# pawanjay176/kzg_rust

Measured on AMD Instinct MI355X. Metric: blobs/sec on verify_blob_kzg_proof_batch (mainnet 4096, batch=64), higher is better.
Workload: dtype u32 limbs (29-bit) / 64-bit accumulate, u8 bytes

## Files before the change

__graft_entry__.py:

```python
import os
import subprocess
import sys

ROOT = os.path.dirname(os.path.abspath(__file__))
if ROOT not in sys.path:
    sys.path.insert(0, ROOT)


def build() -> None:
    env = dict(os.environ)
    subprocess.run(["make", "-C", os.path.join(ROOT, "kzg_rust_amd", "csrc"), "-j5"], check=True, env=env)
    subprocess.run(["make", "-C", os.path.join(ROOT, "oracle")], check=True, env=env)
    native = os.path.join(ROOT, "tests", "native")
    subprocess.run(["g++", "-O2", "-shared", "-fPIC", "-o", os.path.join(native, "libhd_probe.so"), os.path.join(native, "hd_probe.cpp")],
                   check=True, env=env)
    subprocess.run(["g++", "-O2", "-shared", "-fPIC", "-o", os.path.join(native, "liblazy_chain_probe.so"), os.path.join(native, "lazy_chain_probe.cpp")],
                   check=True, env=env)
    subprocess.run(["g++", "-O2", "-shared", "-fPIC", "-o", os.path.join(native, "libmont_columns_probe.so"), os.path.join(native, "mont_columns_probe.cpp")],
                   check=True, env=env)
    subprocess.run(["g++", "-O2", "-std=c++17", "-shared", "-fPIC", "-o", os.path.join(native, "liblc_forms_probe.so"), os.path.join(native, "lc_forms_probe.cpp")],
                   check=True, env=env)
    subprocess.run(["g++", "-std=c++17", "-O2", "-o", os.path.join(native, "cpp_vector_runner"), os.path.join(native, "cpp_vector_runner.cpp"),
                    "-L" + os.path.join(ROOT, "kzg_rust_amd"), "-lkzg355", "-Wl,-rpath," + os.path.join(ROOT, "kzg_rust_amd")], check=True, env=env)
    subprocess.run(["g++", "-std=c++17", "-O2", "-o", os.path.join(native, "cpp_cell_runner"), os.path.join(native, "cpp_cell_runner.cpp"),
                    "-L" + os.path.join(ROOT, "kzg_rust_amd"), "-lkzg355", "-Wl,-rpath," + os.path.join(ROOT, "kzg_rust_amd")], check=True, env=env)
    subprocess.run(["g++", "-std=c++17", "-O2", "-o", os.path.join(native, "cpp_cell_compute_runner"), os.path.join(native, "cpp_cell_compute_runner.cpp"),
                    "-L" + os.path.join(ROOT, "kzg_rust_amd"), "-lkzg355", "-Wl,-rpath," + os.path.join(ROOT, "kzg_rust_amd")], check=True, env=env)
    subprocess.run(["g++", "-std=c++17", "-O2", "-o", os.path.join(native, "cpp_cell_recover_runner"), os.path.join(native, "cpp_cell_recover_runner.cpp"),
                    "-L" + os.path.join(ROOT, "kzg_rust_amd"), "-lkzg355", "-Wl,-rpath," + os.path.join(ROOT, "kzg_rust_amd")], check=True, env=env)
    subprocess.run(["g++", "-std=c++17", "-O2", "-o", os.path.join(native, "cpp_cell_recover_sets_runner"), os.path.join(native, "cpp_cell_recover_sets_runner.cpp"),
                    "-L" + os.path.join(ROOT, "kzg_rust_amd"), "-lkzg355", "-Wl,-rpath," + os.path.join(ROOT, "kzg_rust_amd")], check=True, env=env)
    subprocess.run(["g++", "-std=c++17", "-O2", "-o", os.path.join(native, "cpp_blob_cell_runner"), os.path.join(native, "cpp_blob_cell_runner.cpp"),
                    "-L" + os.path.join(ROOT, "kzg_rust_amd"), "-lkzg355", "-Wl,-rpath," + os.path.join(ROOT, "kzg_rust_amd")], check=True, env=env)
    quad_src, quad_bin = os.path.join(native, "quad_ops_test.hip"), os.path.join(native, "quad_ops_test")
    quad_deps = [quad_src] + [os.path.join(ROOT, "kzg_rust_amd", "csrc", f) for f in ("g1_quad.h", "g1.h", "field.h", "modinv.h", "consts_gen.h")]
    if not os.path.exists(quad_bin) or any(os.path.getmtime(d) > os.path.getmtime(quad_bin) for d in quad_deps):
        subprocess.run(["/opt/rocm/bin/hipcc", "-O3", "-std=c++17", "--offload-arch=gfx950", "-Wno-unused-result", "-o", quad_bin, quad_src], check=True, env=env)
    probe_src, probe_so = os.path.join(native, "gpu_probe.hip"), os.path.join(native, "libgpu_probe.so")
    probe_deps = [probe_src] + [os.path.join(ROOT, "kzg_rust_amd", "csrc", f) for f in ("field.h", "modinv.h", "eval_core.h", "consts_gen.h")]
    if not os.path.exists(probe_so) or any(os.path.getmtime(d) > os.path.getmtime(probe_so) for d in probe_deps):
        subprocess.run(["/opt/rocm/bin/hipcc", "-O3", "-std=c++17", "--offload-arch=gfx950", "-Wno-unused-result", "-shared", "-fPIC", "-o", probe_so, probe_src],
                       check=True, env=env)
    group_src, group_so = os.path.join(native, "gpu_group_probe.hip"), os.path.join(native, "libgpu_group_probe.so")
    group_deps = [group_src] + [os.path.join(ROOT, "kzg_rust_amd", "csrc", f) for f in
                                ("field.h", "modinv.h", "tower.h", "g1.h", "pairing.h", "pairing_coop.h", "pairing_lanes.h", "consts_gen.h")]
    if not os.path.exists(group_so) or any(os.path.getmtime(d) > os.path.getmtime(group_so) for d in group_deps):
        subprocess.run(["/opt/rocm/bin/hipcc", "-O3", "-std=c++17", "--offload-arch=gfx950", "-Wno-unused-result", "-shared", "-fPIC", "-o", group_so, group_src],
                       check=True, env=env)
    import kzg_rust_amd
    from kzg_rust_amd import _lib
    lib = _lib.load()
    for name in _lib.EXPORTED_SYMBOLS:
        getattr(lib, name)
    print("build ok:", lib.kzg355_version().decode())


def smoke() -> None:
    import torch
    assert torch.cuda.is_available(), "smoke() needs a GPU"
    import kzg_rust_amd as kz
    from oracle.oracle import Oracle
    sys.path.insert(0, os.path.join(ROOT, "tests"))
    from synth import random_blob
    golden = os.path.join(ROOT, "tests", "golden")
    g1 = open(os.path.join(golden, "trusted_setup_g1.bin"), "rb").read()
    g2 = open(os.path.join(golden, "trusted_setup_g2.bin"), "rb").read()
    s = kz.Kzg.load_trusted_setup([g1[48 * i:48 * i + 48] for i in range(4096)], [g2[96 * i:96 * i + 96] for i in range(65)])
    o = Oracle()
    os_ = o.load_trusted_setup(g1, g2)
    blobs = [random_blob(1000 + i) for i in range(3)]
    cs = [kz.Kzg.blob_to_kzg_commitment(kz.Blob(b), s) for b in blobs]
    assert [c.to_bytes() for c in cs] == [o.blob_to_kzg_commitment(b, os_) for b in blobs], "commitment mismatch vs oracle"
    ps = [kz.Kzg.compute_blob_kzg_proof(kz.Blob(b), c, s) for b, c in zip(blobs, cs)]
    assert [p.to_bytes() for p in ps] == [o.compute_blob_kzg_proof(b, c.to_bytes(), os_) for b, c in zip(blobs, cs)], "proof mismatch vs oracle"
    ok = kz.Kzg.verify_blob_kzg_proof_batch([kz.Blob(b) for b in blobs], cs, ps, s)
    assert ok is True and o.verify_blob_kzg_proof_batch(blobs, [c.to_bytes() for c in cs], [p.to_bytes() for p in ps], os_) is True
    bad = [ps[1], ps[0], ps[2]]
    assert kz.Kzg.verify_blob_kzg_proof_batch([kz.Blob(b) for b in blobs], cs, bad, s) is False
    s.free()
    o.free_trusted_setup(os_)
    print("smoke ok: commit/prove bit-exact vs oracle, verify batch true/false as expected")


if __name__ == "__main__":
    build()
    if len(sys.argv) > 1 and sys.argv[1] == "smoke":
        smoke()
```

kzg_rust_amd/csrc/eval_core.h:

```cpp
#pragma once
#include "field.h"

namespace kzg {

struct EvalGroup { Fr sa, sb, st; };
constexpr int EVAL_ZPOWERS = 12;
constexpr int EVAL_WAVES = 4;
constexpr int EVAL_TAB_L1 = 0, EVAL_TAB_L2 = 1024, EVAL_TAB_L3 = 1280, EVAL_TAB_L4 = 1344, EVAL_TAB_L5 = 1360, EVAL_TAB_L6 = 1364, EVAL_TAB_GROUPS = 1365;
struct EvalPiece { uint32_t w[4]; };
constexpr int EVAL_TAB_PIECES = ((EVAL_TAB_GROUPS + 63) / 64) * 7 * 64;
KZG_HD constexpr int eval_tab_piece(int e, int q) { return (e / 64) * 7 * 64 + q * 64 + (e % 64); }
KZG_HD void eval_group_pack(EvalPiece p[7], const EvalGroup &g) {
    for (int k = 0; k < 28; k++) p[k / 4].w[k % 4] = k < NFR ? g.sa.l[k] : k < 2 * NFR ? g.sb.l[k - NFR] : k < 3 * NFR ? g.st.l[k - 2 * NFR] : 0u;
}
KZG_HD void eval_group_unpack(EvalGroup &g, const EvalPiece p[7]) {
#pragma unroll
    for (int k = 0; k < 27; k++) (k < NFR ? g.sa.l[k] : k < 2 * NFR ? g.sb.l[k - NFR] : g.st.l[k - 2 * NFR]) = p[k / 4].w[k % 4];
}
KZG_HD constexpr int eval_tab_first(int level) {
    return level == 1 ? EVAL_TAB_L1 : level == 2 ? EVAL_TAB_L2 : level == 3 ? EVAL_TAB_L3 : level == 4 ? EVAL_TAB_L4 : level == 5 ? EVAL_TAB_L5 : EVAL_TAB_L6;
}

template <int K> struct FrMultiple {
    uint32_t l[NFR];
    constexpr FrMultiple() : l{} {
        const uint32_t m[NFR] = FR_MOD_INIT;
        uint64_t c = 0;
        for (int i = 0; i < NFR; i++) { c += (uint64_t)m[i] * (uint32_t)K; l[i] = i < NFR - 1 ? (uint32_t)(c & LMASK) : (uint32_t)c; c >>= LB; }
    }
};
template <int K> KZG_HD void fr_sub_bias(Fr &r, const Fr &a, const Fr &b) {
    constexpr FrMultiple<K> kr;
    int32_t c = 0;
#pragma unroll
    for (int i = 0; i < NFR; i++) {
        const int32_t t = (int32_t)a.l[i] - (int32_t)b.l[i] + (int32_t)kr.l[i] + c;
        if (i < NFR - 1) { c = t >> LB; r.l[i] = (uint32_t)t & LMASK; }
        else r.l[i] = (uint32_t)t;
    }
}

KZG_HD void fr_add_raw(Fr &r, const Fr &a, const Fr &b) {
#pragma unroll
    for (int i = 0; i < NFR; i++) r.l[i] = a.l[i] + b.l[i];
}
template <int K> struct FrMultipleRaw {
    uint32_t l[NFR];
    constexpr FrMultipleRaw() : l{} {
        const FrMultiple<K> n;
        for (int i = 0; i < NFR; i++) l[i] = n.l[i] + (i < NFR - 1 ? (1u << LB) : 0u) - (i > 0 ? 1u : 0u);
    }
};
template <int K> KZG_HD void fr_sub_bias_raw(Fr &r, const Fr &a, const Fr &b) {
    constexpr FrMultipleRaw<K> kr;
#pragma unroll
    for (int i = 0; i < NFR; i++) r.l[i] = a.l[i] - b.l[i] + kr.l[i];
}
KZG_HD void fr_add_sweep(Fr &r, const Fr &a, const Fr &b) {
    uint32_t c = 0;
#pragma unroll
    for (int i = 0; i < NFR; i++) {
        const uint32_t t = a.l[i] + b.l[i] + c;
        if (i < NFR - 1) { c = t >> LB; r.l[i] = t & LMASK; } else r.l[i] = t;
    }
}

template <int K> KZG_HD void eval_node2(Fr &n, const Fr &n0, const Fr &n1, const Fr &zk, const Fr &s) {
    Fr A, B;
    fr_add_raw(A, n0, n1);
    fr_sub_bias_raw<K>(B, n0, n1);
    fr_mul2_lazy(n, A, zk, B, s);
}
KZG_HD void eval_group(Fr &n, const Fr c[4], const Fr &zk, const Fr &zk2, const EvalGroup &g) {
    Fr na, nb;
    eval_node2<2>(na, c[0], c[1], zk, g.sa);
    eval_node2<2>(nb, c[2], c[3], zk, g.sb);
    eval_node2<2>(n, na, nb, zk2, g.st);
}
KZG_HD void eval_group_leaves(Fr &n, Fr &Sp, const uint32_t pw[4][8], const Fr &z, const Fr &z2, const EvalGroup &g) {
    Fr p0, p1, p2, p3, A, B, na, nb, S;
    words_to_limbs<NFR, 8>(p0.l, pw[0]); words_to_limbs<NFR, 8>(p1.l, pw[1]);
    words_to_limbs<NFR, 8>(p2.l, pw[2]); words_to_limbs<NFR, 8>(p3.l, pw[3]);
    fr_add_raw(A, p0, p1); fr_sub_bias_raw<3>(B, p0, p1);
    fr_mul2_lazy(na, A, z, B, g.sa);
    fr_add_raw(S, p2, p3); fr_sub_bias_raw<3>(B, p2, p3);
    fr_mul2_lazy(nb, S, z, B, g.sb);
    fr_add_raw(S, S, A);
    fr_add_sweep(Sp, Sp, S);
    eval_node2<2>(n, na, nb, z2, g.st);
}
KZG_HD void eval_fold(Fr &s) { Fr t; fr_mul_lazy(t, s, fr_one()); s = t; }
KZG_HD void eval_finish(Fr &y, const Fr &ntop, const Fr &Sp, const Fr &z, const Fr &zN) {
    const uint32_t inv4096[NFR] = FR_INV4096_INIT;
    Fr k4096; for (int i = 0; i < NFR; i++) k4096.l[i] = inv4096[i];
    Fr negD, t;
    fr_sub(negD, fr_one(), zN);
    fr_mul2_lazy(t, ntop, z, Sp, negD);
    fr_mul(y, t, k4096);
}

}
```

kzg_rust_amd/csrc/k_verify.hip:

```cpp
#define KZG_FP_MUL_NOINLINE 1
#define KZG_MONT_COLS_FR 1
#include "kernels.h"
#include "sha256_rounds.h"
#include "fr_block.h"

namespace kzg {



constexpr int CH_BLOCKS = 2050;
struct ChallengeReader {
    const uint4 *blob; const uint8_t *cm;
    uint4 line[8];
    uint32_t carry[8];
    __device__ __forceinline__ void prefetch(int b) {
        if (b < 2048 && !(b & 1)) {
            const uint4 *p = blob + 4 * b;
#pragma unroll
            for (int q = 0; q < 8; q++) line[q] = p[q];
        }
    }
    __device__ __forceinline__ void words(uint32_t w[16], int b) {
        if (b == 0) {
            w[0] = 0x4653424cu; w[1] = 0x4f425645u; w[2] = 0x52494659u; w[3] = 0x5f56315fu;
            w[4] = 0; w[5] = 0; w[6] = 0; w[7] = (uint32_t)N_FE;
        } else if (b <= 2048) {
#pragma unroll
            for (int k = 0; k < 8; k++) w[k] = carry[k];
        }
        if (b < 2048) {
            uint4 s0, s1, s2, s3;
            if (b & 1) { s0 = line[4]; s1 = line[5]; s2 = line[6]; s3 = line[7]; }
            else { s0 = line[0]; s1 = line[1]; s2 = line[2]; s3 = line[3]; }
            w[8] = bswap32(s0.x); w[9] = bswap32(s0.y); w[10] = bswap32(s0.z); w[11] = bswap32(s0.w);
            w[12] = bswap32(s1.x); w[13] = bswap32(s1.y); w[14] = bswap32(s1.z); w[15] = bswap32(s1.w);
            carry[0] = bswap32(s2.x); carry[1] = bswap32(s2.y); carry[2] = bswap32(s2.z); carry[3] = bswap32(s2.w);
            carry[4] = bswap32(s3.x); carry[5] = bswap32(s3.y); carry[6] = bswap32(s3.z); carry[7] = bswap32(s3.w);
        } else if (b == 2048) {
            for (int k = 0; k < 8; k++) w[8 + k] = load_be32(cm + 4 * k);
        } else {
            for (int k = 0; k < 4; k++) w[k] = load_be32(cm + 32 + 4 * k);
            w[4] = 0x80000000u;
            for (int k = 5; k < 15; k++) w[k] = 0;
            w[15] = (uint32_t)((32 + BLOB_BYTES + 48) * 8);
        }
    }
};

__device__ __forceinline__ void challenge_finish(const uint32_t hh[8], int i, const uint8_t *cm, const uint8_t *proofs, Fr *z_out, Fr *zpow_out,
        uint8_t *records) {
    const uint32_t dw[8] = {hh[7], hh[6], hh[5], hh[4], hh[3], hh[2], hh[1], hh[0]};
    Fr z; fr_from_words(z, dw);
    z_out[i] = z;
    if (zpow_out) {
        Fr p = z;
#pragma unroll 1
        for (int k = 0; k < EVAL_ZPOWERS; k++) { fr_sqr(p, p); zpow_out[EVAL_ZPOWERS * (size_t)i + k] = p; }
    }
    if (!records) return;
    uint8_t *rec = records + (size_t)RECORD_BYTES * i;
    for (int k = 0; k < 48; k++) rec[k] = cm[k];
    uint8_t zb[32]; fr_to_be32(zb, z);
    for (int k = 0; k < 32; k++) rec[48 + k] = zb[k];
    const uint8_t *pr = proofs + 48 * (size_t)i;
    for (int k = 0; k < 48; k++) rec[112 + k] = pr[k];
}

__global__ void __launch_bounds__(128) k_challenge(const uint8_t *blobs, const uint8_t *commitments, const uint8_t *proofs, int n_total,
                                                    Fr *z_out, Fr *zpow_out, uint8_t *records) {
    __shared__ uint4 wk[2][16][64];
    const int lane = threadIdx.x & 63, role = threadIdx.x >> 6;
    const int i_raw = blockIdx.x * 64 + lane;
    const int i = i_raw < n_total ? i_raw : n_total - 1;
    const uint4 *blob = reinterpret_cast<const uint4 *>(blobs + (size_t)BLOB_BYTES * i);
    const uint8_t *cm = commitments + 48 * (size_t)i;
    static const uint32_t K[64] = {
        0x428a2f98u, 0x71374491u, 0xb5c0fbcfu, 0xe9b5dba5u, 0x3956c25bu, 0x59f111f1u, 0x923f82a4u, 0xab1c5ed5u,
        0xd807aa98u, 0x12835b01u, 0x243185beu, 0x550c7dc3u, 0x72be5d74u, 0x80deb1feu, 0x9bdc06a7u, 0xc19bf174u,
        0xe49b69c1u, 0xefbe4786u, 0x0fc19dc6u, 0x240ca1ccu, 0x2de92c6fu, 0x4a7484aau, 0x5cb0a9dcu, 0x76f988dau,
        0x983e5152u, 0xa831c66du, 0xb00327c8u, 0xbf597fc7u, 0xc6e00bf3u, 0xd5a79147u, 0x06ca6351u, 0x14292967u,
        0x27b70a85u, 0x2e1b2138u, 0x4d2c6dfcu, 0x53380d13u, 0x650a7354u, 0x766a0abbu, 0x81c2c92eu, 0x92722c85u,
        0xa2bfe8a1u, 0xa81a664bu, 0xc24b8b70u, 0xc76c51a3u, 0xd192e819u, 0xd6990624u, 0xf40e3585u, 0x106aa070u,
        0x19a4c116u, 0x1e376c08u, 0x2748774cu, 0x34b0bcb5u, 0x391c0cb3u, 0x4ed8aa4au, 0x5b9cca4fu, 0x682e6ff3u,
        0x748f82eeu, 0x78a5636fu, 0x84c87814u, 0x8cc70208u, 0x90befffau, 0xa4506cebu, 0xbef9a3f7u, 0xc67178f2u};
    ChallengeReader rd; rd.blob = blob; rd.cm = cm;
    auto produce = [&](int b) {
        uint32_t w[16];
        rd.words(w, b);
        rd.prefetch(b + 1);
        uint4 *dst = &wk[b & 1][0][lane];
#pragma unroll
        for (int t = 0; t < 64; t += 4) {
#pragma unroll
            for (int u = 0; u < 4; u++) {
                const int tt = t + u;
                if (tt >= 16) {
                    const uint32_t w15 = w[(tt + 1) & 15], w2 = w[(tt + 14) & 15];
                    const uint32_t s0 = xor3(ror(w15, 7), ror(w15, 18), w15 >> 3);
                    const uint32_t s1 = xor3(ror(w2, 17), ror(w2, 19), w2 >> 10);
                    w[tt & 15] = w[tt & 15] + s0 + w[(tt + 9) & 15] + s1;
                }
            }
            dst[(t >> 2) * 64] = make_uint4(w[t & 15] + K[t], w[(t + 1) & 15] + K[t + 1], w[(t + 2) & 15] + K[t + 2], w[(t + 3) & 15] + K[t + 3]);
        }
    };
    uint32_t h0 = 0x6a09e667u, h1 = 0xbb67ae85u, h2 = 0x3c6ef372u, h3 = 0xa54ff53au, h4 = 0x510e527fu, h5 = 0x9b05688cu, h6 = 0x1f83d9abu, h7 = 0x5be0cd19u;
    if (role == 1) { rd.prefetch(0); produce(0); }
    __syncthreads();
    for (int b = 0; b < CH_BLOCKS; b++) {
        if (role == 0) {
            uint32_t a = h0, bb = h1, c = h2, d = h3, e = h4, f = h5, g = h6, h = h7;
            const uint4 *src = &wk[b & 1][0][lane];
#pragma unroll
            for (int t = 0; t < 64; t += 4) {
                const uint4 q = src[(t >> 2) * 64];
                const uint32_t wv[4] = {q.x, q.y, q.z, q.w};
#pragma unroll
                for (int u = 0; u < 4; u++) {
                    const uint32_t t1 = h + xor3(ror(e, 6), ror(e, 11), ror(e, 25)) + ch3(e, f, g) + wv[u];
                    const uint32_t t2 = xor3(ror(a, 2), ror(a, 13), ror(a, 22)) + maj3(a, bb, c);
                    h = g; g = f; f = e; e = d + t1; d = c; c = bb; bb = a; a = t1 + t2;
                }
            }
            h0 += a; h1 += bb; h2 += c; h3 += d; h4 += e; h5 += f; h6 += g; h7 += h;
        } else if (b + 1 < CH_BLOCKS) {
            produce(b + 1);
        }
        __syncthreads();
    }
    if (role != 0 || i_raw >= n_total) return;
    const uint32_t hh[8] = {h0, h1, h2, h3, h4, h5, h6, h7};
    challenge_finish(hh, i, cm, proofs, z_out, zpow_out, records);
}

constexpr int CH1W_THREADS = 256;
__global__ void __launch_bounds__(CH1W_THREADS) k_challenge_1w(const uint8_t *blobs, const uint8_t *commitments, const uint8_t *proofs, int n_total,
                                                      Fr *z_out, Fr *zpow_out, uint8_t *records) {
    const int i_raw = blockIdx.x * CH1W_THREADS + threadIdx.x;
    const int i = i_raw < n_total ? i_raw : n_total - 1;
    const uint4 *blob = reinterpret_cast<const uint4 *>(blobs + (size_t)BLOB_BYTES * i);
    const uint8_t *cm = commitments + 48 * (size_t)i;
    static const uint32_t K[64] = {
        0x428a2f98u, 0x71374491u, 0xb5c0fbcfu, 0xe9b5dba5u, 0x3956c25bu, 0x59f111f1u, 0x923f82a4u, 0xab1c5ed5u,
        0xd807aa98u, 0x12835b01u, 0x243185beu, 0x550c7dc3u, 0x72be5d74u, 0x80deb1feu, 0x9bdc06a7u, 0xc19bf174u,
        0xe49b69c1u, 0xefbe4786u, 0x0fc19dc6u, 0x240ca1ccu, 0x2de92c6fu, 0x4a7484aau, 0x5cb0a9dcu, 0x76f988dau,
        0x983e5152u, 0xa831c66du, 0xb00327c8u, 0xbf597fc7u, 0xc6e00bf3u, 0xd5a79147u, 0x06ca6351u, 0x14292967u,
        0x27b70a85u, 0x2e1b2138u, 0x4d2c6dfcu, 0x53380d13u, 0x650a7354u, 0x766a0abbu, 0x81c2c92eu, 0x92722c85u,
        0xa2bfe8a1u, 0xa81a664bu, 0xc24b8b70u, 0xc76c51a3u, 0xd192e819u, 0xd6990624u, 0xf40e3585u, 0x106aa070u,
        0x19a4c116u, 0x1e376c08u, 0x2748774cu, 0x34b0bcb5u, 0x391c0cb3u, 0x4ed8aa4au, 0x5b9cca4fu, 0x682e6ff3u,
        0x748f82eeu, 0x78a5636fu, 0x84c87814u, 0x8cc70208u, 0x90befffau, 0xa4506cebu, 0xbef9a3f7u, 0xc67178f2u};
    uint32_t hh[8] = {0x6a09e667u, 0xbb67ae85u, 0x3c6ef372u, 0xa54ff53au, 0x510e527fu, 0x9b05688cu, 0x1f83d9abu, 0x5be0cd19u};
    ChallengeReader rd; rd.blob = blob; rd.cm = cm;
    rd.prefetch(0);
#pragma unroll 1
    for (int b = 0; b < CH_BLOCKS; b++) {
        uint32_t w[16];
        rd.words(w, b);
        rd.prefetch(b + 1);
        uint32_t a = hh[0], bb = hh[1], c = hh[2], d = hh[3], e = hh[4], f = hh[5], g = hh[6], h = hh[7];
#pragma unroll
        for (int t = 0; t < 64; t++) {
            if (t >= 16) {
                const uint32_t w15 = w[(t + 1) & 15], w2 = w[(t + 14) & 15];
                const uint32_t s0 = xor3(ror(w15, 7), ror(w15, 18), w15 >> 3);
                const uint32_t s1 = xor3(ror(w2, 17), ror(w2, 19), w2 >> 10);
                w[t & 15] = w[t & 15] + s0 + w[(t + 9) & 15] + s1;
            }
            const uint32_t t1 = h + xor3(ror(e, 6), ror(e, 11), ror(e, 25)) + ch3(e, f, g) + (w[t & 15] + K[t]);
            const uint32_t t2 = xor3(ror(a, 2), ror(a, 13), ror(a, 22)) + maj3(a, bb, c);
            h = g; g = f; f = e; e = d + t1; d = c; c = bb; bb = a; a = t1 + t2;
        }
        hh[0] += a; hh[1] += bb; hh[2] += c; hh[3] += d; hh[4] += e; hh[5] += f; hh[6] += g; hh[7] += h;
    }
    if (i_raw >= n_total) return;
    challenge_finish(hh, i, cm, proofs, z_out, zpow_out, records);
}

__global__ void __launch_bounds__(64) k_challenge_from_digest(const uint8_t *digests, const uint8_t *commitments, const uint8_t *proofs, int n_total,
                                                              Fr *z_out, Fr *zpow_out, uint8_t *records) {
    const int i = blockIdx.x * 64 + threadIdx.x;
    if (i >= n_total) return;
    uint32_t hh[8];
#pragma unroll
    for (int k = 0; k < 8; k++) hh[k] = load_be32(digests + 32 * (size_t)i + 4 * k);
    challenge_finish(hh, i, commitments + 48 * (size_t)i, proofs, z_out, zpow_out, records);
}

__device__ __forceinline__ void eval_issue_tile_loads(const uint4 *blob_step, uint4 *tile, int lane) {
#pragma unroll
    for (int q = 0; q < 8; q++) {
        const int g = 8 * q + (lane >> 3), s = lane & 7;
        __builtin_amdgcn_global_load_lds((const void __attribute__((address_space(1))) *)(blob_step + 8 * g + (s ^ (g & 7))),
                                         (void __attribute__((address_space(3))) *)(tile + 64 * q), 16, 0, 0);
    }
}
__device__ __forceinline__ void eval_tab_load(EvalPiece p[7], const EvalPiece *tab, int e) {
    const uint4 *src = reinterpret_cast<const uint4 *>(tab);
#pragma unroll
    for (int q = 0; q < 7; q++) { const uint4 v = src[eval_tab_piece(e, q)]; p[q].w[0] = v.x; p[q].w[1] = v.y; p[q].w[2] = v.z; p[q].w[3] = v.w; }
}
__device__ __forceinline__ void eval_park(uint32_t *hx, int entry, const Fr &h) {
#pragma unroll
    for (int k = 0; k < NFR; k++) hx[NFR * entry + k] = h.l[k];
}
__device__ __forceinline__ void eval_children(Fr c[4], const uint32_t *hx, int node) {
    __builtin_amdgcn_fence(__ATOMIC_RELEASE, "workgroup"); __builtin_amdgcn_wave_barrier(); __builtin_amdgcn_fence(__ATOMIC_ACQUIRE, "workgroup");
    const uint4 *src = reinterpret_cast<const uint4 *>(hx + 4 * NFR * node);
    uint32_t w[4 * NFR];
#pragma unroll
    for (int q = 0; q < NFR; q++) { const uint4 v = src[q]; w[4 * q] = v.x; w[4 * q + 1] = v.y; w[4 * q + 2] = v.z; w[4 * q + 3] = v.w; }
#pragma unroll
    for (int e = 0; e < 4; e++)
#pragma unroll
        for (int k = 0; k < NFR; k++) c[e].l[k] = w[NFR * e + k];
    __builtin_amdgcn_fence(__ATOMIC_RELEASE, "workgroup"); __builtin_amdgcn_wave_barrier();
}
__global__ void __launch_bounds__(64 * EVAL_WAVES, 2) k_eval(const uint8_t *blobs, const Fr *z_in, const Fr *zpow, const EvalPiece *tab, int n_total,
                                                          int n_per_group, Fr *y_out, uint8_t *records, int *err) {
    __shared__ uint4 tiles[EVAL_WAVES][512];
    __shared__ __attribute__((aligned(16))) uint32_t hxs[EVAL_WAVES][256 * NFR];
    const int wid = __builtin_amdgcn_readfirstlane((int)(threadIdx.x >> 6)), lane = threadIdx.x & 63;
    const int blob_raw = blockIdx.x * EVAL_WAVES + wid;
    const int blob_i = blob_raw < n_total ? blob_raw : n_total - 1;
    uint4 *tile = tiles[wid];
    uint32_t *hx = hxs[wid];
    const uint4 *blob = reinterpret_cast<const uint4 *>(blobs + (size_t)BLOB_BYTES * blob_i);
    eval_issue_tile_loads(blob, tile, lane);
    const Fr z = z_in[blob_i];
    const Fr *zp = zpow + EVAL_ZPOWERS * (size_t)blob_i;
    const Fr z2 = zp[0];
    __shared__ uint32_t zls[EVAL_WAVES][4 * NFR];
    const uint32_t zl_word = reinterpret_cast<const uint32_t *>(zp + 1)[lane < 4 * NFR ? lane : 0];
    Fr h2[4], Sp = fr_zero();
    bool bad = false;
    constexpr int STEPS = N_FE / 4 / 64;
    EvalPiece g_next[7];
    eval_tab_load(g_next, tab, EVAL_TAB_L1 + lane);
#pragma unroll 1
    for (int it = 0; it < STEPS; it++) {
        __builtin_amdgcn_s_waitcnt(0);
        __builtin_amdgcn_fence(__ATOMIC_ACQUIRE, "workgroup");
        if (it == 0 && lane < 4 * NFR) zls[wid][lane] = zl_word;
        uint4 cur[8];
#pragma unroll
        for (int j = 0; j < 8; j++) cur[j] = tile[8 * lane + (j ^ (lane & 7))];
        EvalGroup g1; eval_group_unpack(g1, g_next);
        __builtin_amdgcn_fence(__ATOMIC_RELEASE, "workgroup"); __builtin_amdgcn_wave_barrier();
        if (it + 1 < STEPS) eval_issue_tile_loads(blob + 512 * (it + 1), tile, lane);
        const int e_l1 = EVAL_TAB_L1 + ((it + 1) & (STEPS - 1)) * 64 + lane, e_l2 = EVAL_TAB_L2 + 64 * (it >> 2) + lane;
        eval_tab_load(g_next, tab, (it & 3) == 3 ? e_l2 : e_l1);
        uint32_t pw[4][8];
#pragma unroll
        for (int e = 0; e < 4; e++) {
            const uint4 a = cur[2 * e], b = cur[2 * e + 1];
            pw[e][7] = bswap32(a.x); pw[e][6] = bswap32(a.y); pw[e][5] = bswap32(a.z); pw[e][4] = bswap32(a.w);
            pw[e][3] = bswap32(b.x); pw[e][2] = bswap32(b.y); pw[e][1] = bswap32(b.z); pw[e][0] = bswap32(b.w);
        }
        const uint32_t top = max(max(pw[0][7], pw[1][7]), max(pw[2][7], pw[3][7]));
        if (top >= FR_MOD_TOP_WORD) {
#pragma unroll 1
            for (int e = 0; e < 4; e++) bad = bad || !fr_words_canonical(pw[e]);
        }
        Fr h;
        eval_group_leaves(h, Sp, pw, z, z2, g1);
        eval_park(hx, 64 * (it & 3) + lane, h);
        if ((it & 3) == 3) {
            Fr c[4];
            eval_children(c, hx, lane);
            EvalGroup g2; eval_group_unpack(g2, g_next);
            eval_tab_load(g_next, tab, it + 1 < STEPS ? e_l1 : EVAL_TAB_L3 + lane);
            Fr z4, z8;
#pragma unroll
            for (int k = 0; k < NFR; k++) { z4.l[k] = zls[wid][k]; z8.l[k] = zls[wid][NFR + k]; }
            Fr r2; eval_group(r2, c, z4, z8, g2);
#pragma unroll
            for (int a = 0; a < 4; a++) if ((it >> 2) == a) h2[a] = r2;
        }
    }
    if (bad && blob_raw < n_total) atomicOr(&err[blob_i / n_per_group], ERR_NONCANONICAL_FR);
    Fr c[4], h;
#pragma unroll
    for (int a = 0; a < 4; a++) eval_park(hx, 64 * a + lane, h2[a]);
    eval_children(c, hx, lane);
    EvalGroup g3; eval_group_unpack(g3, g_next);
    Fr z16, z32;
#pragma unroll
    for (int k = 0; k < NFR; k++) { z16.l[k] = zls[wid][2 * NFR + k]; z32.l[k] = zls[wid][3 * NFR + k]; }
    eval_group(h, c, z16, z32, g3);
    const int b = lane >> 4, u = lane & 15;
    const int mine_raw = blockIdx.x * EVAL_WAVES + b, mine = mine_raw < n_total ? mine_raw : n_total - 1;
    const Fr *zq = zpow + EVAL_ZPOWERS * (size_t)mine;
    Fr zt[7];
#pragma unroll
    for (int k = 0; k < 7; k++) zt[k] = zq[5 + k];
    const Fr zmine = z_in[mine];
    EvalPiece gp4[7], gp5[7], gp6[7];
    eval_tab_load(gp4, tab, EVAL_TAB_L4 + u); eval_tab_load(gp5, tab, EVAL_TAB_L5 + (lane & 3)); eval_tab_load(gp6, tab, EVAL_TAB_L6);
    eval_fold(Sp);
#pragma unroll
    for (int off = 32; off > 0; off >>= 1) { const Fr o = fr_shfl_down(Sp, off); fr_add_lazy(Sp, Sp, o); }
    eval_park(hx, lane, h);
    if (lane == 0) eval_park(hx, 64, Sp);
    __syncthreads();
    if (wid != 0) return;
    Fr Sb;
#pragma unroll
    for (int k = 0; k < NFR; k++) Sb.l[k] = hxs[b][NFR * 64 + k];
    eval_children(c, hxs[b], u);
    EvalGroup gt; eval_group_unpack(gt, gp4);
    eval_group(h, c, zt[0], zt[1], gt);
    uint32_t *hx0 = hxs[0];
    eval_park(hx0, lane, h);
    eval_children(c, hx0, 4 * b + (lane & 3));
    eval_group_unpack(gt, gp5);
    eval_group(h, c, zt[2], zt[3], gt);
    if (u < 4) eval_park(hx0, 4 * b + u, h);
    eval_children(c, hx0, b);
    eval_group_unpack(gt, gp6);
    eval_group(h, c, zt[4], zt[5], gt);
    Fr y; eval_finish(y, h, Sb, zmine, zt[6]);
    if (u == 0 && mine_raw < n_total) {
        if (records) {
            uint32_t yw[8]; limbs_to_words<NFR, 8>(yw, y.l);
            uint8_t *rec = records + (size_t)RECORD_BYTES * mine + 80;
#pragma unroll
            for (int i = 0; i < 8; i++) {
                const uint32_t v = yw[7 - i];
                rec[4 * i] = (uint8_t)(v >> 24); rec[4 * i + 1] = (uint8_t)(v >> 16); rec[4 * i + 2] = (uint8_t)(v >> 8); rec[4 * i + 3] = (uint8_t)v;
            }
        }
        if (y_out) {
            const uint32_t r2[NFR] = FR_R2_INIT;
            Fr R2; for (int i = 0; i < NFR; i++) R2.l[i] = r2[i];
            Fr ym; fr_mul(ym, y, R2);
            y_out[mine] = ym;
        }
    }
}

__global__ void __launch_bounds__(64) k_rhash_lanes(const uint8_t *records, int n, int groups, uint32_t *digests, int n_fe) {
    const int g = blockIdx.x * 64 + threadIdx.x;
    if (g >= groups) return;
    const uint8_t *rec = records + (size_t)RECORD_BYTES * n * g;
    const uint32_t total_words = 8u + 40u * (uint32_t)n;
    const uint32_t nblocks = (total_words * 4u + 9u + 63u) / 64u;
    const uint64_t bits = (uint64_t)total_words * 32u;
    uint32_t hs[8] = {0x6a09e667u, 0xbb67ae85u, 0x3c6ef372u, 0xa54ff53au, 0x510e527fu, 0x9b05688cu, 0x1f83d9abu, 0x5be0cd19u};
#pragma unroll 1
    for (uint32_t b = 0; b < nblocks; b++) {
        uint32_t w[16];
        if (b >= 1u && 16u * b + 16u <= total_words) {
            const uint4 *p = reinterpret_cast<const uint4 *>(rec + 64u * (size_t)b - 32u);
#pragma unroll
            for (int q = 0; q < 4; q++) {
                const uint4 v = p[q];
                w[4 * q] = bswap32(v.x); w[4 * q + 1] = bswap32(v.y); w[4 * q + 2] = bswap32(v.z); w[4 * q + 3] = bswap32(v.w);
            }
        } else {
#pragma unroll
            for (int t = 0; t < 16; t++) {
                const uint32_t idx = 16u * b + (uint32_t)t;
                uint32_t v;
                if (idx < 8u) {
                    const uint32_t hdr[8] = {0x52434b5au, 0x47424154u, 0x43485f5fu, 0x5f56315fu, 0u, (uint32_t)n_fe, 0u, (uint32_t)n};
                    v = hdr[idx];
                } else if (idx < total_words) v = bswap32(reinterpret_cast<const uint32_t *>(rec)[idx - 8u]);
                else if (idx == total_words) v = 0x80000000u;
                else if (idx == 16u * nblocks - 2u) v = (uint32_t)(bits >> 32);
                else if (idx == 16u * nblocks - 1u) v = (uint32_t)bits;
                else v = 0u;
                w[t] = v;
            }
        }
        uint32_t a = hs[0], bb = hs[1], c = hs[2], d = hs[3], e = hs[4], f = hs[5], gg = hs[6], h = hs[7];
#pragma unroll
        for (int t = 0; t < 64; t++) {
            if (t >= 16) {
                const uint32_t w15 = w[(t + 1) & 15], w2 = w[(t + 14) & 15];
                const uint32_t s0 = xor3(ror(w15, 7), ror(w15, 18), w15 >> 3);
                const uint32_t s1 = xor3(ror(w2, 17), ror(w2, 19), w2 >> 10);
                w[t & 15] = w[t & 15] + s0 + w[(t + 9) & 15] + s1;
            }
            const uint32_t t1 = h + xor3(ror(e, 6), ror(e, 11), ror(e, 25)) + ch3(e, f, gg) + w[t & 15] + SHA_K[t];
            const uint32_t t2 = xor3(ror(a, 2), ror(a, 13), ror(a, 22)) + maj3(a, bb, c);
            h = gg; gg = f; f = e; e = d + t1; d = c; c = bb; bb = a; a = t1 + t2;
        }
        hs[0] += a; hs[1] += bb; hs[2] += c; hs[3] += d; hs[4] += e; hs[5] += f; hs[6] += gg; hs[7] += h;
    }
#pragma unroll
    for (int k = 0; k < 8; k++) digests[8 * (size_t)g + k] = hs[7 - k];
}

__global__ void __launch_bounds__(256) k_rpowers(const uint8_t *records, int n, int groups, int check_zy, uint32_t *scal_a, uint32_t *scal_b,
                                                  uint32_t *scal_c, int *err, int n_fe, int have_digest) {
    __shared__ uint32_t wk_all[4][64][64];
    __shared__ uint32_t digest_all[4][8];
    const int wid = threadIdx.x >> 6, lane = threadIdx.x & 63;
    const int g_raw = blockIdx.x * (int)(blockDim.x >> 6) + wid;
    if (g_raw >= groups) return;
    const int g = g_raw;
    const bool live = true;
    uint32_t (*wk)[64] = wk_all[wid];
    uint32_t *digest = digest_all[wid];
    const uint8_t *rec = records + (size_t)RECORD_BYTES * n * g;
    Fr r = fr_one();
    if (n > 1 && have_digest) {
        uint32_t dw[8];
#pragma unroll
        for (int k = 0; k < 8; k++) dw[k] = scal_c[8 * (size_t)g + k];
        fr_from_words(r, dw);
    } else if (n > 1) {
        const uint32_t total_words = 8u + 40u * (uint32_t)n;
        const uint32_t nblocks = (total_words * 4u + 9u + 63u) / 64u;
        const uint64_t bits = (uint64_t)total_words * 32u;
        uint32_t h0 = 0x6a09e667u, h1 = 0xbb67ae85u, h2 = 0x3c6ef372u, h3 = 0xa54ff53au, h4 = 0x510e527fu, h5 = 0x9b05688cu, h6 = 0x1f83d9abu, h7 = 0x5be0cd19u;
        for (uint32_t b0 = 0; b0 < nblocks; b0 += 64) {
            const uint32_t b = b0 + (uint32_t)lane;
            if (b < nblocks) {
                uint32_t w[16];
#pragma unroll
                for (int t = 0; t < 16; t++) {
                    const uint32_t idx = 16u * b + (uint32_t)t;
                    uint32_t v;
                    if (idx < 8u) {
                        const uint32_t hdr[8] = {0x52434b5au, 0x47424154u, 0x43485f5fu, 0x5f56315fu, 0u, (uint32_t)n_fe, 0u, (uint32_t)n};
                        v = hdr[idx];
                    } else if (idx < total_words) v = bswap32(reinterpret_cast<const uint32_t *>(rec)[idx - 8u]);
                    else if (idx == total_words) v = 0x80000000u;
                    else if (idx == 16u * nblocks - 2u) v = (uint32_t)(bits >> 32);
                    else if (idx == 16u * nblocks - 1u) v = (uint32_t)bits;
                    else v = 0u;
                    w[t] = v;
                }
#pragma unroll
                for (int t = 0; t < 64; t++) {
                    if (t >= 16) {
                        const uint32_t w15 = w[(t + 1) & 15], w2 = w[(t + 14) & 15];
                        const uint32_t s0 = xor3(ror(w15, 7), ror(w15, 18), w15 >> 3);
                        const uint32_t s1 = xor3(ror(w2, 17), ror(w2, 19), w2 >> 10);
                        w[t & 15] = w[t & 15] + s0 + w[(t + 9) & 15] + s1;
                    }
                    wk[t][lane] = w[t & 15] + SHA_K[t];
                }
            }
            SHA_WAVE_SYNC();
            if (lane == 0) {
                const uint32_t cnt = nblocks - b0 < 64u ? nblocks - b0 : 64u;
#pragma unroll 1
                for (uint32_t q = 0; q < cnt; q++) {
                    uint32_t a = h0, bb = h1, c = h2, d = h3, e = h4, f = h5, gg = h6, h = h7;
#pragma unroll
                    for (int t = 0; t < 64; t++) {
                        const uint32_t t1 = h + xor3(ror(e, 6), ror(e, 11), ror(e, 25)) + ch3(e, f, gg) + wk[t][q];
                        const uint32_t t2 = xor3(ror(a, 2), ror(a, 13), ror(a, 22)) + maj3(a, bb, c);
                        h = gg; gg = f; f = e; e = d + t1; d = c; c = bb; bb = a; a = t1 + t2;
                    }
                    h0 += a; h1 += bb; h2 += c; h3 += d; h4 += e; h5 += f; h6 += gg; h7 += h;
                }
            }
            SHA_WAVE_SYNC();
        }
        if (lane == 0) { digest[0] = h7; digest[1] = h6; digest[2] = h5; digest[3] = h4; digest[4] = h3; digest[5] = h2; digest[6] = h1; digest[7] = h0; }
        SHA_WAVE_SYNC();
        uint32_t dw[8];
#pragma unroll
        for (int k = 0; k < 8; k++) dw[k] = digest[k];
        fr_from_words(r, dw);
    }
    Fr pw = fr_one(), r64 = r;
#pragma unroll 1
    for (int bit = 5; bit >= 0; bit--) {
        Fr t;
        fr_sqr(pw, pw);
        fr_mul(t, pw, r);
        fr_select(pw, (lane >> bit) & 1, pw, t);
        fr_sqr(r64, r64);
    }
    Fr csum = fr_zero();
    bool bad = false;
#pragma unroll 1
    for (int i = lane; i < n; i += 64) {
        uint32_t zw[8], yw[8];
        be32_to_words(zw, rec + (size_t)RECORD_BYTES * i + 48);
        be32_to_words(yw, rec + (size_t)RECORD_BYTES * i + 80);
        if (check_zy) bad = bad || !fr_words_canonical(zw) || !fr_words_canonical(yw);
        Fr z, y, t; fr_from_words(z, zw); fr_from_words(y, yw);
        uint32_t *pa = scal_a + 8 * ((size_t)g * n + i), *pb = scal_b + 8 * ((size_t)g * n + i);
        uint32_t ow[8];
        fr_to_words(ow, pw); if (live) for (int k = 0; k < 8; k++) pa[k] = ow[k];
        fr_mul(t, pw, z); fr_to_words(ow, t); if (live) for (int k = 0; k < 8; k++) pb[k] = ow[k];
        fr_mul(t, pw, y); fr_add(csum, csum, t);
        fr_mul(pw, pw, r64);
    }
#pragma unroll
    for (int off = 32; off > 0; off >>= 1) { Fr o = fr_shfl_down(csum, off); fr_add(csum, csum, o); }
    if (lane == 0 && live) {
        uint32_t ow[8]; fr_to_words(ow, csum);
        for (int k = 0; k < 8; k++) scal_c[8 * (size_t)g + k] = ow[k];
    }
    if (bad && live) atomicOr(&err[g], ERR_NONCANONICAL_FR);
}

__global__ void __launch_bounds__(64) k_pairing(const PairPt *pair_pts, const LineCoeff *lines, const int *lines_inf, int groups, int *ok) {
    const int g = blockIdx.x * blockDim.x + threadIdx.x;
    if (g >= groups) return;
    G1Affine p1, p2; pairpt_to_affine(p1, pair_pts[2 * (size_t)g]); pairpt_to_affine(p2, pair_pts[2 * (size_t)g + 1]);
    if (lines_inf[2]) p1 = g1a_inf();
    if (lines_inf[0]) p2 = g1a_inf();
    Fp12 f;
    miller_loop_pair(f, lines + 2 * N_LINES, p1, lines, p2);
    ok[g] = final_exp_is_one(f) ? 1 : 0;
}

void launch_challenges(const uint8_t *d_blobs, const uint8_t *d_commitments, const uint8_t *d_proofs, int n_total, Fr *d_z, Fr *d_zpow, uint8_t *d_records,
                       hipStream_t st, int form) {
    if (n_total <= 0) return;
    const int wgs = (n_total + 63) / 64;
    if (form == 2 || (form == 0 && wgs <= 512)) hipLaunchKernelGGL(k_challenge, dim3(wgs), dim3(128), 0, st, d_blobs, d_commitments, d_proofs, n_total, d_z,
            d_zpow, d_records);
    else hipLaunchKernelGGL(k_challenge_1w, dim3((n_total + CH1W_THREADS - 1) / CH1W_THREADS), dim3(CH1W_THREADS), 0, st, d_blobs, d_commitments, d_proofs,
            n_total, d_z, d_zpow, d_records);
}
void launch_challenges_from_digests(const uint8_t *d_digests, const uint8_t *d_commitments, const uint8_t *d_proofs, int n_total, Fr *d_z, Fr *d_zpow,
                                    uint8_t *d_records, hipStream_t st) {
    if (n_total <= 0) return;
    hipLaunchKernelGGL(k_challenge_from_digest, dim3((n_total + 63) / 64), dim3(64), 0, st, d_digests, d_commitments, d_proofs, n_total, d_z, d_zpow,
            d_records);
}
void launch_eval(const uint8_t *d_blobs, const Fr *d_z, const Fr *d_zpow, DeviceTables t, int n_total, int n_per_group, Fr *d_y, uint8_t *d_records, int *d_err,
                 hipStream_t st) {
    if (n_total <= 0) return;
    hipLaunchKernelGGL(k_eval, dim3((n_total + EVAL_WAVES - 1) / EVAL_WAVES), dim3(64 * EVAL_WAVES), 0, st, d_blobs, d_z, d_zpow, t.eval_tab, n_total,
            n_per_group,
                       d_y, d_records, d_err);
}
void launch_rpowers(const uint8_t *d_records, int n_per_group, int groups, int check_zy, uint32_t *d_scal_a, uint32_t *d_scal_b,
                    uint32_t *d_scal_c, int *d_err, hipStream_t st, int n_fe, int lanes_from, int have_digest) {
    if (groups <= 0) return;
    const int wpw = groups > 512 ? 4 : 1;
    const int lanes = (!have_digest && n_per_group > 1 && groups >= lanes_from) ? 1 : 0;
    if (lanes) hipLaunchKernelGGL(k_rhash_lanes, dim3((groups + 63) / 64), dim3(64), 0, st, d_records, n_per_group, groups, d_scal_c, n_fe);
    hipLaunchKernelGGL(k_rpowers, dim3((groups + wpw - 1) / wpw), dim3(64 * wpw), 0, st, d_records, n_per_group, groups, check_zy, d_scal_a, d_scal_b,
            d_scal_c, d_err, n_fe, lanes || have_digest);
}
void launch_pairing_lane(const PairPt *d_pair_pts, DeviceTables t, int groups, int *d_ok, hipStream_t st) {
    if (groups <= 0) return;
    hipLaunchKernelGGL(k_pairing, dim3((groups + 63) / 64), dim3(64), 0, st, d_pair_pts, t.lines, t.lines_inf, groups, d_ok);
}

}
```

Baseline: 4.685 million.

## Split eval leaf work around tile prefetch and defer running-sum carry sweep

Restructures the k_eval main loop so the first leaf pair is computed before the next tile's global loads are issued. Explicit waitcnt masks and scheduling barriers make LDS waits separate from VMEM waits, and workgroup-scope fences are replaced with wavefront-scope ordering. The per-iteration carry-propagating running sum is replaced by a 64-bit per-limb column accumulator that is swept once after the loop. The intent is to hide load latency and drop per-iteration sweep cost, at the risk of using more registers and depending on hand-written waitcnt encodings being correct.

```diff
diff --git a/__graft_entry__.py b/__graft_entry__.py
--- a/__graft_entry__.py
+++ b/__graft_entry__.py
@@ -13,6 +13,8 @@
     subprocess.run(["make", "-C", os.path.join(ROOT, "oracle")], check=True, env=env)
     native = os.path.join(ROOT, "tests", "native")
     subprocess.run(["g++", "-O2", "-shared", "-fPIC", "-o", os.path.join(native, "libhd_probe.so"), os.path.join(native, "hd_probe.cpp")],
+                   check=True, env=env)
+    subprocess.run(["g++", "-O2", "-shared", "-fPIC", "-o", os.path.join(native, "libeval_sum_probe.so"), os.path.join(native, "eval_sum_probe.cpp")],
                    check=True, env=env)
     subprocess.run(["g++", "-O2", "-shared", "-fPIC", "-o", os.path.join(native, "liblazy_chain_probe.so"), os.path.join(native, "lazy_chain_probe.cpp")],
                    check=True, env=env)
diff --git a/kzg_rust_amd/csrc/eval_core.h b/kzg_rust_amd/csrc/eval_core.h
--- a/kzg_rust_amd/csrc/eval_core.h
+++ b/kzg_rust_amd/csrc/eval_core.h
@@ -77,17 +77,34 @@
     eval_node2<2>(nb, c[2], c[3], zk, g.sb);
     eval_node2<2>(n, na, nb, zk2, g.st);
 }
+KZG_HD void eval_leaf_pair(Fr &n, Fr &A, const uint32_t pa[8], const uint32_t pb[8], const Fr &z, const Fr &s) {
+    Fr p0, p1, B;
+    words_to_limbs<NFR, 8>(p0.l, pa); words_to_limbs<NFR, 8>(p1.l, pb);
+    fr_add_raw(A, p0, p1); fr_sub_bias_raw<3>(B, p0, p1);
+    fr_mul2_lazy(n, A, z, B, s);
+}
 KZG_HD void eval_group_leaves(Fr &n, Fr &Sp, const uint32_t pw[4][8], const Fr &z, const Fr &z2, const EvalGroup &g) {
-    Fr p0, p1, p2, p3, A, B, na, nb, S;
-    words_to_limbs<NFR, 8>(p0.l, pw[0]); words_to_limbs<NFR, 8>(p1.l, pw[1]);
-    words_to_limbs<NFR, 8>(p2.l, pw[2]); words_to_limbs<NFR, 8>(p3.l, pw[3]);
-    fr_add_raw(A, p0, p1); fr_sub_bias_raw<3>(B, p0, p1);
-    fr_mul2_lazy(na, A, z, B, g.sa);
-    fr_add_raw(S, p2, p3); fr_sub_bias_raw<3>(B, p2, p3);
-    fr_mul2_lazy(nb, S, z, B, g.sb);
+    Fr A, na, nb, S;
+    eval_leaf_pair(na, A, pw[0], pw[1], z, g.sa);
+    eval_leaf_pair(nb, S, pw[2], pw[3], z, g.sb);
     fr_add_raw(S, S, A);
     fr_add_sweep(Sp, Sp, S);
     eval_node2<2>(n, na, nb, z2, g.st);
+}
+struct FrSum { uint64_t c[NFR]; };
+KZG_HD FrSum fr_sum_zero() { FrSum s; for (int i = 0; i < NFR; i++) s.c[i] = 0; return s; }
+KZG_HD void fr_sum_add(FrSum &s, const Fr &A, const Fr &S) {
+#pragma unroll
+    for (int i = 0; i < NFR; i++) s.c[i] += (uint64_t)(A.l[i] + S.l[i]);
+}
+KZG_HD uint64_t fr_sum_column(const FrSum &s, int i) { return s.c[i]; }
+KZG_HD void fr_sum_sweep(Fr &r, const FrSum &s) {
+    uint64_t c = 0;
+#pragma unroll
+    for (int i = 0; i < NFR; i++) {
+        const uint64_t t = fr_sum_column(s, i) + c;
+        if (i < NFR - 1) { c = t >> LB; r.l[i] = (uint32_t)t & LMASK; } else r.l[i] = (uint32_t)t;
+    }
 }
 KZG_HD void eval_fold(Fr &s) { Fr t; fr_mul_lazy(t, s, fr_one()); s = t; }
 KZG_HD void eval_finish(Fr &y, const Fr &ntop, const Fr &Sp, const Fr &z, const Fr &zN) {
diff --git a/kzg_rust_amd/csrc/k_verify.hip b/kzg_rust_amd/csrc/k_verify.hip
--- a/kzg_rust_amd/csrc/k_verify.hip
+++ b/kzg_rust_amd/csrc/k_verify.hip
@@ -203,8 +203,12 @@
 #pragma unroll
     for (int k = 0; k < NFR; k++) hx[NFR * entry + k] = h.l[k];
 }
+__device__ __forceinline__ void eval_wave_order() {
+    __builtin_amdgcn_fence(__ATOMIC_RELEASE, "wavefront"); __builtin_amdgcn_wave_barrier(); __builtin_amdgcn_fence(__ATOMIC_ACQUIRE, "wavefront");
+}
+constexpr int EVAL_WAIT_VMCNT0 = 0x0F70, EVAL_WAIT_LGKMCNT0 = 0xC07F, EVAL_WAIT_VMCNT0_LGKMCNT0 = 0x0070;
 __device__ __forceinline__ void eval_children(Fr c[4], const uint32_t *hx, int node) {
-    __builtin_amdgcn_fence(__ATOMIC_RELEASE, "workgroup"); __builtin_amdgcn_wave_barrier(); __builtin_amdgcn_fence(__ATOMIC_ACQUIRE, "workgroup");
+    eval_wave_order();
     const uint4 *src = reinterpret_cast<const uint4 *>(hx + 4 * NFR * node);
     uint32_t w[4 * NFR];
 #pragma unroll
@@ -213,7 +217,15 @@
     for (int e = 0; e < 4; e++)
 #pragma unroll
         for (int k = 0; k < NFR; k++) c[e].l[k] = w[NFR * e + k];
-    __builtin_amdgcn_fence(__ATOMIC_RELEASE, "workgroup"); __builtin_amdgcn_wave_barrier();
+    eval_wave_order();
+}
+__device__ __forceinline__ void eval_pin(Fr &x) {
+#pragma unroll
+    for (int k = 0; k < NFR; k++) asm volatile("" : "+v"(x.l[k]));
+}
+__device__ __forceinline__ void eval_words(uint32_t w[8], const uint4 &a, const uint4 &b) {
+    w[7] = bswap32(a.x); w[6] = bswap32(a.y); w[5] = bswap32(a.z); w[4] = bswap32(a.w);
+    w[3] = bswap32(b.x); w[2] = bswap32(b.y); w[1] = bswap32(b.z); w[0] = bswap32(b.w);
 }
 __global__ void __launch_bounds__(64 * EVAL_WAVES, 2) k_eval(const uint8_t *blobs, const Fr *z_in, const Fr *zpow, const EvalPiece *tab, int n_total,
                                                           int n_per_group, Fr *y_out, uint8_t *records, int *err) {
@@ -231,42 +243,51 @@
     const Fr z2 = zp[0];
     __shared__ uint32_t zls[EVAL_WAVES][4 * NFR];
     const uint32_t zl_word = reinterpret_cast<const uint32_t *>(zp + 1)[lane < 4 * NFR ? lane : 0];
-    Fr h2[4], Sp = fr_zero();
+    Fr h2[4];
+    FrSum Ssum = fr_sum_zero();
     bool bad = false;
     constexpr int STEPS = N_FE / 4 / 64;
     EvalPiece g_next[7];
     eval_tab_load(g_next, tab, EVAL_TAB_L1 + lane);
 #pragma unroll 1
     for (int it = 0; it < STEPS; it++) {
-        __builtin_amdgcn_s_waitcnt(0);
-        __builtin_amdgcn_fence(__ATOMIC_ACQUIRE, "workgroup");
+        __builtin_amdgcn_s_waitcnt(EVAL_WAIT_VMCNT0_LGKMCNT0);
+        eval_wave_order();
         if (it == 0 && lane < 4 * NFR) zls[wid][lane] = zl_word;
         uint4 cur[8];
 #pragma unroll
-        for (int j = 0; j < 8; j++) cur[j] = tile[8 * lane + (j ^ (lane & 7))];
+        for (int j = 0; j < 4; j++) cur[j] = tile[8 * lane + (j ^ (lane & 7))];
+#pragma unroll
+        for (int j = 4; j < 8; j++) cur[j] = tile[8 * lane + (j ^ (lane & 7))];
         EvalGroup g1; eval_group_unpack(g1, g_next);
-        __builtin_amdgcn_fence(__ATOMIC_RELEASE, "workgroup"); __builtin_amdgcn_wave_barrier();
+        uint32_t pw[4][8];
+        eval_words(pw[0], cur[0], cur[1]); eval_words(pw[1], cur[2], cur[3]);
+        Fr A, S, na, nb;
+        eval_leaf_pair(na, A, pw[0], pw[1], z, g1.sa);
+        eval_pin(na);
+        __builtin_amdgcn_sched_barrier(0);
+        __builtin_amdgcn_s_waitcnt(EVAL_WAIT_LGKMCNT0);
+        eval_wave_order();
         if (it + 1 < STEPS) eval_issue_tile_loads(blob + 512 * (it + 1), tile, lane);
         const int e_l1 = EVAL_TAB_L1 + ((it + 1) & (STEPS - 1)) * 64 + lane, e_l2 = EVAL_TAB_L2 + 64 * (it >> 2) + lane;
         eval_tab_load(g_next, tab, (it & 3) == 3 ? e_l2 : e_l1);
-        uint32_t pw[4][8];
-#pragma unroll
-        for (int e = 0; e < 4; e++) {
-            const uint4 a = cur[2 * e], b = cur[2 * e + 1];
-            pw[e][7] = bswap32(a.x); pw[e][6] = bswap32(a.y); pw[e][5] = bswap32(a.z); pw[e][4] = bswap32(a.w);
-            pw[e][3] = bswap32(b.x); pw[e][2] = bswap32(b.y); pw[e][1] = bswap32(b.z); pw[e][0] = bswap32(b.w);
-        }
+        __builtin_amdgcn_sched_barrier(0);
+        eval_words(pw[2], cur[4], cur[5]); eval_words(pw[3], cur[6], cur[7]);
         const uint32_t top = max(max(pw[0][7], pw[1][7]), max(pw[2][7], pw[3][7]));
         if (top >= FR_MOD_TOP_WORD) {
 #pragma unroll 1
             for (int e = 0; e < 4; e++) bad = bad || !fr_words_canonical(pw[e]);
         }
+        eval_leaf_pair(nb, S, pw[2], pw[3], z, g1.sb);
+        fr_sum_add(Ssum, A, S);
         Fr h;
-        eval_group_leaves(h, Sp, pw, z, z2, g1);
+        eval_node2<2>(h, na, nb, z2, g1.st);
         eval_park(hx, 64 * (it & 3) + lane, h);
         if ((it & 3) == 3) {
             Fr c[4];
             eval_children(c, hx, lane);
+            __builtin_amdgcn_s_waitcnt(EVAL_WAIT_VMCNT0);
+            __builtin_amdgcn_sched_barrier(0);
             EvalGroup g2; eval_group_unpack(g2, g_next);
             eval_tab_load(g_next, tab, it + 1 < STEPS ? e_l1 : EVAL_TAB_L3 + lane);
             Fr z4, z8;
@@ -296,6 +317,7 @@
     const Fr zmine = z_in[mine];
     EvalPiece gp4[7], gp5[7], gp6[7];
     eval_tab_load(gp4, tab, EVAL_TAB_L4 + u); eval_tab_load(gp5, tab, EVAL_TAB_L5 + (lane & 3)); eval_tab_load(gp6, tab, EVAL_TAB_L6);
+    Fr Sp; fr_sum_sweep(Sp, Ssum);
     eval_fold(Sp);
 #pragma unroll
     for (int off = 32; off > 0; off >>= 1) { const Fr o = fr_shfl_down(Sp, off); fr_add_lazy(Sp, Sp, o); }
```

After: 4.699 million, median of 2. About the same (+0.3%).
